# hzykent/LiDAL

Measured on AMD Instinct MI355X. Metric: voxels/sec SPVCNN fwd+bwd @120k pts, higher is better.
Workload: dtype bf16; 1 GPU; spvcnn train step (train.py:127-140: fwd + CE + bwd + Adam), 5 scans x ~120k pts per GPU, 0.05 m voxels, kernel maps rebuilt every step (each step builds the next step's coordinate tables on a second stream; variants.inline_geometry: built inside the forward pass); parallelism=dp1

## Files before the change

### lidal_amd/csrc/voxel.hip

```cpp
#include <cstring>


#include "common.h"

using namespace lidal;

namespace {

typedef __attribute__((ext_vector_type(4))) __bf16 bf16x4_t;

__device__ __forceinline__ float4 ld4(const float* p) { return *reinterpret_cast<const float4*>(p); }
__device__ __forceinline__ float4 ld4(const __bf16* p) {
  bf16x4_t v = *reinterpret_cast<const bf16x4_t*>(p);
  return make_float4((float)v[0], (float)v[1], (float)v[2], (float)v[3]);
}
__device__ __forceinline__ void st4(float* p, float4 v) { *reinterpret_cast<float4*>(p) = v; }
__device__ __forceinline__ void st4(__bf16* p, float4 v) {
  bf16x4_t o;
  o[0] = (__bf16)v.x; o[1] = (__bf16)v.y; o[2] = (__bf16)v.z; o[3] = (__bf16)v.w;
  *reinterpret_cast<bf16x4_t*>(p) = o;
}

template <int VEC>
__device__ __forceinline__ void ldv(const float* p, float (&a)[VEC]) {
// ... 393 lines not shown
  float inv = 1.f;
  if (!DEVOX) { int cv = counts[v]; inv = cv > 0 ? (float)cv : 1.f; }
  float acc[VEC];
#pragma unroll
  for (int u = 0; u < VEC; ++u) acc[u] = 0.f;
  auto add = [&](const float (&x)[VEC], float sc) {
#pragma unroll
    for (int u = 0; u < VEC; ++u) acc[u] += DEVOX ? sc * x[u] : x[u] / inv;
  };
  int64_t j = beg;
  for (; j + 3 < end; j += 4) {
    int e[4]; float sc[4]; float x[4][VEC];
#pragma unroll
    for (int u = 0; u < 4; ++u) e[u] = order[j + u];
#pragma unroll
    for (int u = 0; u < 4; ++u) {
      sc[u] = DEVOX ? w[e[u]] : 1.f;
      ldv<VEC>(src + (int64_t)(DEVOX ? (e[u] >> 3) : e[u]) * c + l * VEC, x[u]);
    }
#pragma unroll
    for (int u = 0; u < 4; ++u) add(x[u], sc[u]);
  }
  for (; j < end; ++j) {
    const int e = order[j];
    float x[VEC];
    ldv<VEC>(src + (int64_t)(DEVOX ? (e >> 3) : e) * c + l * VEC, x);
    add(x, DEVOX ? w[e] : 1.f);
  }
  stv<VEC>(out + v * c + l * VEC, acc);
}

template <typename T>
__global__ void __launch_bounds__(256) segment_fold_kernel(const float* __restrict__ partial,
                                                           T* __restrict__ out, int64_t m, int c,
                                                           int parts) {
  const int cv = c / 4;
  int64_t t = (int64_t)blockIdx.x * 256 + threadIdx.x;
  if (t >= m * cv) return;
  int64_t v = t / cv;
  int j = (int)(t - v * cv) * 4;
  float4 a = ld4(partial + (v * parts) * c + j);
  for (int p = 1; p < parts; ++p) {
    float4 b = ld4(partial + (v * parts + p) * c + j);
    a.x += b.x; a.y += b.y; a.z += b.z; a.w += b.w;
  }
  st4(out + v * c + j, a);
}

static inline int row_lanes(int c, int vec) {
  const int need = (c + vec - 1) / vec;
  int lpr = 4;
  while (lpr < need) lpr <<= 1;
  return lpr > 64 ? 64 : lpr;
}
static inline int segment_vec(int c, int esz) { return (esz == 2 && c % 8 == 0) ? 8 : 4; }
static inline int segment_parts(int64_t n_entries, int64_t m, int c, int esz) {
  if (m <= 0) return 0;
  const int lpr = row_lanes(c, segment_vec(c, esz));
  const int64_t rpw = 64 / lpr, avg = n_entries / m;
  if (avg < 20 * rpw && (m >= 65536 || avg < 8 * rpw)) return 0;
  const int64_t waves = (avg + 16 * rpw - 1) / (16 * rpw);
  int parts = 1;
  while (parts < 4 && (int64_t)parts * 4 < waves) parts <<= 1;
  return parts;
}

constexpr int64_t GROUP_MAX_AVG = 32, GROUP_MAX_AVG_FEW = 12, GROUP_MANY_VOXELS = 65536;

template <typename T, int VEC, bool DEVOX>
void launch_group(const T* src, const int* order, const int64_t* seg_ptr, const float* w, const int* counts,
                  T* out, int64_t m, int c, hipStream_t s) {
  const int need = (c + VEC - 1) / VEC;
#define LIDAL_GROUP(LPR)                                                                               \
  segment_sum_group_kernel<T, LPR, VEC, DEVOX><<<(unsigned)cdiv(m, 256 / LPR), 256, 0, s>>>(src, order, seg_ptr, w, \
                                                                                          counts, out, m, c)
  if (need <= 4) LIDAL_GROUP(4);
  else if (need <= 8) LIDAL_GROUP(8);
  else if (need <= 16) LIDAL_GROUP(16);
  else if (need <= 32) LIDAL_GROUP(32);
  else LIDAL_GROUP(64);
#undef LIDAL_GROUP
}

template <typename T, bool DEVOX>
int launch_segment_sum(const T* src, const int* order, const int64_t* seg_ptr, const float* w,
                       const int* counts, T* out, int64_t m, int c, int64_t n_entries, void* ws,
                       int64_t ws_bytes, hipStream_t s) {
  LIDAL_REQUIRE(c <= 64 * segment_vec(c, (int)sizeof(T)), "segment_sum: at most %d channels per row for this element type",
                64 * segment_vec(c, (int)sizeof(T)));
  if (m > 0 && n_entries / m <= (m >= GROUP_MANY_VOXELS ? GROUP_MAX_AVG : GROUP_MAX_AVG_FEW)) {
    if (sizeof(T) == 2 && c % 8 == 0) launch_group<T, 8, DEVOX>(src, order, seg_ptr, w, counts, out, m, c, s);
    else launch_group<T, 4, DEVOX>(src, order, seg_ptr, w, counts, out, m, c, s);
    LIDAL_CHECK_LAUNCH("segment_sum_group");
    return 0;
  }
  const int parts = segment_parts(n_entries, m, c, (int)sizeof(T));
  float* partial = (float*)ws;
  if (parts > 1)
    LIDAL_REQUIRE(ws != nullptr && ws_bytes >= (int64_t)m * parts * c * 4, "segment_sum workspace too small");
  const bool wide = segment_vec(c, (int)sizeof(T)) == 8;
  const int lpr = row_lanes(c, wide ? 8 : 4);
#define LIDAL_SEG(LPR, VEC)                                                                              \
  do {                                                                                                   \
    if (parts == 0)                                                                                      \
      segment_sum_kernel<T, LPR, VEC, DEVOX><<<(unsigned)cdiv(m, 4), 256, 0, s>>>(src, order, seg_ptr, w, counts, \
                                                                                 out, m, c);             \
    else                                                                                                 \
      segment_sum_wg_kernel<T, LPR, VEC, DEVOX><<<(unsigned)(m * parts), 256, 0, s>>>(                   \
          src, order, seg_ptr, w, counts, out, partial, m, c, parts);                                    \
  } while (0)
  if (wide) {
    if (lpr <= 4) LIDAL_SEG(4, 8); else if (lpr == 8) LIDAL_SEG(8, 8); else if (lpr == 16) LIDAL_SEG(16, 8);
    else if (lpr == 32) LIDAL_SEG(32, 8); else LIDAL_SEG(64, 8);
  } else {
    if (lpr <= 8) LIDAL_SEG(8, 4); else if (lpr == 16) LIDAL_SEG(16, 4); else if (lpr == 32) LIDAL_SEG(32, 4);
    else LIDAL_SEG(64, 4);
  }
#undef LIDAL_SEG
  LIDAL_CHECK_LAUNCH("segment_sum");
  if (parts > 1) {
    segment_fold_kernel<T><<<(unsigned)cdiv(m * (c / 4), 256), 256, 0, s>>>(partial, out, m, c, parts);
    LIDAL_CHECK_LAUNCH("segment_fold");
  }
  return 0;
}

template <typename T, int LPR, int VEC>
__global__ void __launch_bounds__(256) devox_cell_sums_kernel(const T* __restrict__ g, const int* __restrict__ vorder,
                                                              const int64_t* __restrict__ vseg,
                                                              const float* __restrict__ w8, float* __restrict__ cs,
                                                              int64_t m, int c) {
  constexpr int RPW = 64 / LPR;
  __shared__ float red[3][8][LPR * VEC];
  const int lane = threadIdx.x & 63, wave = threadIdx.x >> 6;
  const int l = lane % LPR, grp = lane / LPR;
  const int64_t cell = blockIdx.x;
  const int64_t beg = vseg[cell], end = vseg[cell + 1];
  const int64_t quarter = (end - beg + 3) / 4;
  int64_t b0 = beg + (int64_t)wave * quarter, b1 = b0 + quarter;
  if (b0 > end) b0 = end;
  if (b1 > end) b1 = end;
  float acc[8][VEC];
#pragma unroll
  for (int k = 0; k < 8; ++k)
#pragma unroll
    for (int q = 0; q < VEC; ++q) acc[k][q] = 0.f;
  auto add = [&](const float (&x)[VEC], const float4& wa, const float4& wb) {
    const float wv[8] = {wa.x, wa.y, wa.z, wa.w, wb.x, wb.y, wb.z, wb.w};
#pragma unroll
    for (int k = 0; k < 8; ++k)
      if (wv[k] != 0.f) {
#pragma unroll
        for (int q = 0; q < VEC; ++q) acc[k][q] += wv[k] * x[q];
      }
  };
  for (int64_t base = b0; base < b1; base += 64) {
    const int cnt = (int)((b1 - base < 64) ? (b1 - base) : 64);
    const int mine = lane < cnt ? vorder[base + lane] : 0;
    int ib = 0;
    for (; ib + 4 * RPW <= cnt; ib += 4 * RPW) {
      const int i = ib + grp;
      int p[4]; float x[4][VEC]; float4 wa[4], wb[4];
#pragma unroll
      for (int u = 0; u < 4; ++u) p[u] = __shfl(mine, i + u * RPW, 64);
#pragma unroll
      for (int u = 0; u < 4; ++u) {
        ldv<VEC>(g + (int64_t)p[u] * c + VEC * l, x[u]);
        wa[u] = ld4(w8 + (int64_t)p[u] * 8); wb[u] = ld4(w8 + (int64_t)p[u] * 8 + 4);
      }
#pragma unroll
      for (int u = 0; u < 4; ++u) add(x[u], wa[u], wb[u]);
    }
    for (; ib < cnt; ib += RPW) {
      const int i = ib + grp;
      const bool ok = i < cnt;
      const int p0 = __shfl(mine, ok ? i : 0, 64);
      if (ok) {
        float x0[VEC];
        ldv<VEC>(g + (int64_t)p0 * c + VEC * l, x0);
        add(x0, ld4(w8 + (int64_t)p0 * 8), ld4(w8 + (int64_t)p0 * 8 + 4));
      }
    }
  }
#pragma unroll
  for (int off = LPR; off < 64; off <<= 1) {
#pragma unroll
    for (int k = 0; k < 8; ++k)
#pragma unroll
      for (int q = 0; q < VEC; ++q) acc[k][q] += __shfl_xor(acc[k][q], off, 64);
  }
  if (wave > 0 && grp == 0) {
#pragma unroll
    for (int k = 0; k < 8; ++k)
#pragma unroll
      for (int q = 0; q < VEC; ++q) red[wave - 1][k][l * VEC + q] = acc[k][q];
  }
  __syncthreads();
  if (wave == 0 && grp == 0) {
#pragma unroll
    for (int k = 0; k < 8; ++k) {
      float* dst = cs + ((int64_t)cell * 8 + k) * c + VEC * l;
#pragma unroll
      for (int q = 0; q < VEC; q += 4) {
        float o[4];
#pragma unroll
        for (int e = 0; e < 4; ++e)
          o[e] = ((acc[k][q + e] + red[0][k][l * VEC + q + e]) + red[1][k][l * VEC + q + e]) + red[2][k][l * VEC + q + e];
        st4(dst + q, make_float4(o[0], o[1], o[2], o[3]));
      }
    }
  }
}

template <typename T>
__global__ void __launch_bounds__(256) devox_cell_fold_kernel(const float* __restrict__ cs, const int* __restrict__ corder,
                                                              const int64_t* __restrict__ cseg, T* __restrict__ gin,
                                                              int64_t m, int c) {
  const int cv = c / 4;
  const int64_t t = (int64_t)blockIdx.x * 256 + threadIdx.x;
  if (t >= m * cv) return;
  const int64_t v = t / cv;
  const int jj = (int)(t - v * cv) * 4;
  float4 a = make_float4(0.f, 0.f, 0.f, 0.f);
  for (int64_t i = cseg[v]; i < cseg[v + 1]; ++i) {
    const float4 b = ld4(cs + (int64_t)corder[i] * c + jj);
    a.x += b.x; a.y += b.y; a.z += b.z; a.w += b.w;
  }
  st4(gin + v * c + jj, a);
}

template <typename T>
int launch_devox_cells(const T* g, const int* vorder, const int64_t* vseg, const float* w8, const int* corder,
                       const int64_t* cseg, T* gin, int64_t m, int c, float* cs, hipStream_t s) {
  constexpr int VEC = 16 / (int)sizeof(T);
  const int lpr = c / VEC;
#define LIDAL_CELLS(LPR) devox_cell_sums_kernel<T, LPR, VEC><<<(unsigned)m, 256, 0, s>>>(g, vorder, vseg, w8, cs, m, c)
  if (lpr == 4) LIDAL_CELLS(4); else if (lpr == 8) LIDAL_CELLS(8); else if (lpr == 16) LIDAL_CELLS(16);
  else if (lpr == 32) LIDAL_CELLS(32); else LIDAL_CELLS(64);
#undef LIDAL_CELLS
  LIDAL_CHECK_LAUNCH("devoxelize_bwd_cells(sums)");
  devox_cell_fold_kernel<T><<<(unsigned)cdiv(m * (c / 4), 256), 256, 0, s>>>(cs, corder, cseg, gin, m, c);
  LIDAL_CHECK_LAUNCH("devoxelize_bwd_cells(fold)");
  return 0;
}

}

#define DISPATCH_VEC(kernel, c, total_rows, ...)                                             \
  do {                                                                                       \
    if ((c) % 4 == 0) {                                                                      \
      int64_t t__ = (total_rows) * ((c) / 4);                                                \
      kernel<4><<<(unsigned)cdiv(t__, 256), 256, 0, s>>>(__VA_ARGS__);                       \
    } else {                                                                                 \
      int64_t t__ = (total_rows) * (c);                                                      \
      kernel<1><<<(unsigned)cdiv(t__, 256), 256, 0, s>>>(__VA_ARGS__);                       \
    }                                                                                        \
  } while (0)

#define DISPATCH_TVEC(kernel, T, c, total_rows, ...)                                         \
  do {                                                                                       \
    if (sizeof(T) == 2 && (c) % 8 == 0) {                  \
      int64_t t__ = (total_rows) * ((c) / 8);                                                \
      kernel<T, 8><<<(unsigned)cdiv(t__, 256), 256, 0, s>>>(__VA_ARGS__);                    \
    } else if ((c) % 4 == 0) {                                                                      \
      int64_t t__ = (total_rows) * ((c) / 4);                                                \
      kernel<T, 4><<<(unsigned)cdiv(t__, 256), 256, 0, s>>>(__VA_ARGS__);                    \
    } else {                                                                                 \
      int64_t t__ = (total_rows) * (c);                                                      \
      kernel<T, 1><<<(unsigned)cdiv(t__, 256), 256, 0, s>>>(__VA_ARGS__);                    \
    }                                                                                        \
  } while (0)

extern "C" int lidal_count(const int32_t* idx, int64_t n, int32_t* out, int64_t m, void* stream) {
  hipStream_t s = (hipStream_t)stream;
  if (m > 0) LIDAL_HIP(hipMemsetAsync(out, 0, 4 * m, s));
  if (n == 0 || m == 0) return 0;
  count_kernel<<<(unsigned)cdiv(n, 256), 256, 0, s>>>(idx, n, out, m);
  LIDAL_CHECK_LAUNCH("lidal_count");
  return 0;
}

extern "C" int lidal_voxelize_fwd(const float* feat, const int32_t* idx, const int32_t* counts,
                                  float* out, int64_t n, int64_t m, int c, void* stream) {
  hipStream_t s = (hipStream_t)stream;
  if (m > 0 && c > 0) LIDAL_HIP(hipMemsetAsync(out, 0, 4 * m * c, s));
  if (n == 0 || m == 0 || c == 0) return 0;
  DISPATCH_VEC(voxelize_fwd_kernel, c, n, feat, idx, counts, out, n, m, c);
  LIDAL_CHECK_LAUNCH("lidal_voxelize_fwd");
  return 0;
}

namespace {
template <typename T, int VEC>
__global__ void __launch_bounds__(256) voxelize_1to1_kernel(const T* __restrict__ feat, const int* __restrict__ idx,
                                                            T* __restrict__ out, int64_t n, int c) {
  const int cv = c / VEC;
  const int64_t t = (int64_t)blockIdx.x * blockDim.x + threadIdx.x;
  if (t >= n * cv) return;
  const int64_t i = t / cv;
  const int j = (int)(t - i * cv) * VEC;
  const int pos = idx[i];
  if (pos < 0 || pos >= n) return;
  const T* src = feat + i * c + j;
  T* dst = out + (int64_t)pos * c + j;
#pragma unroll
  for (int v = 0; v < VEC; ++v) dst[v] = src[v];
}
}

extern "C" int lidal_voxelize_fwd_1to1(const void* feat, const int32_t* idx, void* out, int64_t n, int c,
                                       int dtype, void* stream) {
  hipStream_t s = (hipStream_t)stream;
  if (n == 0 || c == 0) return 0;
  if (dtype == LIDAL_F32)
    DISPATCH_TVEC(voxelize_1to1_kernel, float, c, n, (const float*)feat, idx, (float*)out, n, c);
  else if (dtype == LIDAL_BF16)
    DISPATCH_TVEC(voxelize_1to1_kernel, __bf16, c, n, (const __bf16*)feat, idx, (__bf16*)out, n, c);
  else { set_error("voxelize_fwd_1to1: bad dtype %d", dtype); return 2; }
  LIDAL_CHECK_LAUNCH("lidal_voxelize_fwd_1to1");
  return 0;
}

extern "C" int lidal_voxelize_bwd(const void* gout, const int32_t* idx, const int32_t* counts,
                                  const void* residual, void* gin, int64_t n, int64_t m, int c,
                                  int dtype, void* stream) {
  hipStream_t s = (hipStream_t)stream;
  if (n == 0 || c == 0) return 0;
  if (dtype == LIDAL_F32)
    DISPATCH_TVEC(voxelize_bwd_kernel, float, c, n, (const float*)gout, idx, counts,
                  (const float*)residual, (float*)gin, n, m, c);
  else if (dtype == LIDAL_BF16)
    DISPATCH_TVEC(voxelize_bwd_kernel, __bf16, c, n, (const __bf16*)gout, idx, counts,
                  (const __bf16*)residual, (__bf16*)gin, n, m, c);
  else { set_error("voxelize_bwd: bad dtype %d", dtype); return 2; }
  LIDAL_CHECK_LAUNCH("lidal_voxelize_bwd");
  return 0;
}

extern "C" int lidal_devoxelize_fwd(const void* feat, const int32_t* idx, const float* w,
                                    void* out, int64_t n, int64_t m, int c, int dtype,
                                    void* stream) {
  hipStream_t s = (hipStream_t)stream;
  if (n == 0 || c == 0) return 0;
  if (dtype == LIDAL_F32)
    DISPATCH_TVEC(devoxelize_fwd_kernel, float, c, n, (const float*)feat, idx, w, (float*)out, n, m, c);
  else if (dtype == LIDAL_BF16)
    DISPATCH_TVEC(devoxelize_fwd_kernel, __bf16, c, n, (const __bf16*)feat, idx, w, (__bf16*)out, n, m, c);
  else { set_error("devoxelize_fwd: bad dtype %d", dtype); return 2; }
  LIDAL_CHECK_LAUNCH("lidal_devoxelize_fwd");
  return 0;
}

extern "C" int lidal_devoxelize_bwd(const float* gout, const int32_t* idx, const float* w,
                                    float* gin, int64_t n, int64_t m, int c, void* stream) {
  hipStream_t s = (hipStream_t)stream;
  if (m > 0 && c > 0) LIDAL_HIP(hipMemsetAsync(gin, 0, 4 * m * c, s));
  if (n == 0 || m == 0 || c == 0) return 0;
  DISPATCH_VEC(devoxelize_bwd_kernel, c, n, gout, idx, w, gin, n, m, c);
  LIDAL_CHECK_LAUNCH("lidal_devoxelize_bwd");
  return 0;
}

extern "C" int lidal_ti_weights(const float* coords, int cstride, const int64_t* idx, int64_t n,
                                float scale, float* w, int32_t* idx32, void* stream) {
  hipStream_t s = (hipStream_t)stream;
  if (n == 0) return 0;
  LIDAL_REQUIRE(cstride >= 3, "ti_weights: coords need >= 3 columns");
  ti_weights_kernel<<<(unsigned)cdiv(n, 256), 256, 0, s>>>(coords, cstride, idx, n, scale, w, idx32);
  LIDAL_CHECK_LAUNCH("lidal_ti_weights");
  return 0;
}

static int64_t inv_tmp_bytes(int64_t q) { return sort_pairs_ws_bytes(q); }

extern "C" int64_t lidal_invlist_workspace_bytes(int64_t n_entries) {
  int64_t q = n_entries > 0 ? n_entries : 1;
  return 2 * align_up(4 * q, 256) + align_up(4 * q, 256) + align_up(inv_tmp_bytes(q), 256) + 256;
}

extern "C" int lidal_invlist_build(const int32_t* idx, const float* w, int64_t n_entries, int64_t m,
                                   int32_t* order, int64_t* seg_ptr, void* ws, int64_t ws_bytes,
                                   void* stream) {
  hipStream_t s = (hipStream_t)stream;
  LIDAL_REQUIRE(m >= 0 && m < 0x7FFFFFFF, "invlist: bad voxel count");
  if (n_entries == 0) {
    LIDAL_HIP(hipMemsetAsync(seg_ptr, 0, 8 * (m + 1), s));
    return 0;
  }
  LIDAL_REQUIRE(ws_bytes >= lidal_invlist_workspace_bytes(n_entries), "invlist workspace too small");
  int64_t q = n_entries;
  unsigned* keys = (unsigned*)ws;
  unsigned* skeys = (unsigned*)((char*)ws + align_up(4 * q, 256));
  int* vals = (int*)((char*)ws + 2 * align_up(4 * q, 256));
  void* tmp = (char*)ws + 3 * align_up(4 * q, 256);
  inv_keys_kernel<<<(unsigned)cdiv(q, 256), 256, 0, s>>>(idx, w, q, m, keys, vals);
  LIDAL_CHECK_LAUNCH("inv_keys");
  int bits = 1;
  while ((1ll << bits) <= m) ++bits;
  if (int rc = sort_pairs_u32(keys, vals, skeys, order, q, bits, tmp, inv_tmp_bytes(q), s)) return rc;
  inv_segptr_kernel<<<(unsigned)cdiv(m + 1, 256), 256, 0, s>>>(skeys, q, m, seg_ptr);
  LIDAL_CHECK_LAUNCH("inv_segptr");
  return 0;
}

extern "C" int64_t lidal_segment_workspace_bytes(int64_t n_entries, int64_t m, int c) {
  int parts = segment_parts(n_entries, m, c, 2), parts4 = segment_parts(n_entries, m, c, 4);
  if (parts4 > parts) parts = parts4;
  return parts > 1 ? (int64_t)m * parts * c * 4 : 0;
}

extern "C" int lidal_voxelize_fwd_sorted(const void* feat, const int32_t* order,
                                         const int64_t* seg_ptr, const int32_t* counts, void* out,
                                         int64_t m, int c, int dtype, int64_t n_entries, void* ws,
                                         int64_t ws_bytes, void* stream) {
  if (m == 0 || c == 0) return 0;
  LIDAL_REQUIRE(c % 4 == 0, "voxelize_fwd_sorted: channels must be a multiple of 4");
  if (dtype == LIDAL_F32)
    return launch_segment_sum<float, false>((const float*)feat, order, seg_ptr, nullptr, counts,
                                            (float*)out, m, c, n_entries, ws, ws_bytes,
                                            (hipStream_t)stream);
  if (dtype == LIDAL_BF16)
    return launch_segment_sum<__bf16, false>((const __bf16*)feat, order, seg_ptr, nullptr, counts,
                                             (__bf16*)out, m, c, n_entries, ws, ws_bytes,
                                             (hipStream_t)stream);
  set_error("voxelize_fwd_sorted: bad dtype %d", dtype);
  return 2;
}

extern "C" int64_t lidal_devoxelize_bwd_cells_workspace_bytes(int64_t m, int c) { return m * 8 * (int64_t)c * 4; }
extern "C" int lidal_devoxelize_bwd_cells(const void* gout, const int32_t* vorder, const int64_t* vseg, const float* w8,
                                          const int32_t* corder, const int64_t* cseg, void* gin, int64_t m, int c,
                                          int dtype, void* ws, int64_t ws_bytes, void* stream) {
  if (m == 0 || c == 0) return 0;
  const int vec = dtype == LIDAL_F32 ? 4 : 8;
  const int lpr = c / vec;
  LIDAL_REQUIRE(dtype == LIDAL_F32 || dtype == LIDAL_BF16, "devoxelize_bwd_cells: bad dtype %d", dtype);
  LIDAL_REQUIRE(c % vec == 0 && lpr >= 4 && lpr <= 64 && (lpr & (lpr - 1)) == 0,
                "devoxelize_bwd_cells: %d channels (a power of two of 16-byte steps, 4 .. 64 of them)", c);
  LIDAL_REQUIRE(ws != nullptr && ws_bytes >= lidal_devoxelize_bwd_cells_workspace_bytes(m, c), "devoxelize_bwd_cells ws too small");
  if (dtype == LIDAL_F32)
    return launch_devox_cells<float>((const float*)gout, vorder, vseg, w8, corder, cseg, (float*)gin, m, c, (float*)ws,
                                     (hipStream_t)stream);
  return launch_devox_cells<__bf16>((const __bf16*)gout, vorder, vseg, w8, corder, cseg, (__bf16*)gin, m, c, (float*)ws,
                                    (hipStream_t)stream);
}

extern "C" int lidal_devoxelize_bwd_sorted(const void* gout, const int32_t* order,
                                           const int64_t* seg_ptr, const float* w, void* gin,
                                           int64_t m, int c, int dtype, int64_t n_entries, void* ws,
                                           int64_t ws_bytes, void* stream) {
  if (m == 0 || c == 0) return 0;
  LIDAL_REQUIRE(c % 4 == 0, "devoxelize_bwd_sorted: channels must be a multiple of 4");
  if (dtype == LIDAL_F32)
    return launch_segment_sum<float, true>((const float*)gout, order, seg_ptr, w, nullptr,
                                           (float*)gin, m, c, n_entries, ws, ws_bytes,
                                           (hipStream_t)stream);
  if (dtype == LIDAL_BF16)
    return launch_segment_sum<__bf16, true>((const __bf16*)gout, order, seg_ptr, w, nullptr,
                                            (__bf16*)gin, m, c, n_entries, ws, ws_bytes,
                                            (hipStream_t)stream);
  set_error("devoxelize_bwd_sorted: bad dtype %d", dtype);
  return 2;
}
```

### lidal_amd/network/plan.py

```python
import array
import ctypes
import os
import struct

import torch

from .. import backend as B
from ..nn.functional import conv as _C
from ..nn.functional import norm as _N
from ..nn.functional import devoxelize as _DV
from ..nn.functional.invlist import inverse_lists
from ..nn.functional.voxelize import _index32

__all__ = ['planned_forward', 'enabled', 'COUNTERS']

ENABLED = os.environ.get('LIDAL_PLAN', '1') != '0'
BN_SUMS = None

OP_CONV_WEIGHT_IMAGE_BATCH, OP_CONV_APPLY_IMAGE, OP_CONV_DGRAD_BN_SUMS, OP_CONV_WGRAD = 1, 2, 3, 4
OP_BN_TRAIN_FWD, OP_BN_TRAIN_FWD_TILES, OP_BN_BWD, OP_BN_BWD_TILES, OP_BN_EVAL_FWD, OP_BN_FOLD = 5, 6, 7, 8, 9, 10
OP_COLSUM, OP_ADD_RELU_FWD, OP_ADD_RELU_BWD, OP_VOXELIZE_FWD_1TO1, OP_VOXELIZE_FWD_SORTED = 11, 12, 13, 14, 15
OP_VOXELIZE_BWD, OP_DEVOXELIZE_FWD, OP_DEVOXELIZE_BWD_SORTED, OP_CE_FWD, OP_CE_BWD = 16, 17, 18, 19, 20
OP_COPY2D, OP_ADD2D, OP_TRANSPOSE_F32, OP_CAST_ROWS_BF16, OP_VIEW_MEAN_SOFTMAX = 21, 22, 23, 24, 25
OP_FORK_SIDE, OP_JOIN_SIDE, OP_CONV_APPLY_IMAGE_WS, OP_CONV_DGRAD_BN_SUMS_WS = 26, 27, 28, 29
# ... 878 lines not shown
        self.w += (OP_CONV_WGRAD | flag, x, g, n, n, 0, self.koff[n], 0, gw, sc, slabs, 1, ca, cb, wcode)
        self.nops += 1
        if not direct:
            self.w += (OP_TRANSPOSE_F32 | flag, gw, cb, self.slot(c.w), ca, c.co)
            self.nops += 1
        if not need_gx:
            return 0
        gx = self.galloc(n * ca * self.esz)
        self.w += (OP_CONV_APPLY_IMAGE | branch, g, c.img_b, 0, 0, 0, gx, n, n, cb, ca, 1, 0, self.code, 0, 0, 0, 0, 0)
        self.nops += 1
        return gx

    def b_colsum(self, g, n, c, out, flag=0):
        nb = _bn_ws(n, c) + 12 * c
        self.w += (OP_COLSUM | flag, g, self.code, n, c, out, self.scratch(nb, flag), nb)
        self.nops += 1

    def b_conv_bn(self, cb, g, g_stride, n_in, n_out, tables, need_gx=True, ci=None):
        c, r = cb
        x, x1, mean, invstd = self.saved[id(cb)]
        dx = self.b_bn(r, x1, n_out, mean, invstd, g, g_stride)
        if c.transposed:
            rules, table, n_gin, kflip = tables[6:8], tables[0:3], n_in, 0
        elif c.strided:
            rules, table, n_gin, kflip = tables[6:8], tables[3:6], n_in, 0
        else:
            rules, table, n_gin, kflip = tables[3:8], tables[0:3], n_in, 1
        self.b_wgrad(c, x, n_in, dx, n_out, rules, ci)
        if not need_gx:
            return 0
        return self.b_dgrad(c, dx, n_out, table, n_gin, kflip)[0]

    def b_res(self, r, g, n, k3):
        x, x1, mean1, inv1, y1, x2, mean2, inv2, out, xs, means, invs = self.saved[id(r)]
        co = r.c2.co
        gm = self.galloc(n * co * self.esz)
        part2 = parts = nb = 0
        sums2 = sumss = nparts = 0
        if _N.tail_tiles(n, self.dtype):
            nparts = int(B.lib().lidal_bn_tail_parts(n, co, self.code))
            sums2 = self.galloc(co * nparts * 8)
            sumss = self.galloc(co * nparts * 8) if r.cs is not None else 0
            self.w += (OP_ADD_RELU_BWD_BN_TILE_SUMS, out, g, gm, self.code, n, co, x2, mean2, inv2, sums2,
                       xs if sumss else 0, means if sumss else 0, invs if sumss else 0, sumss, nparts)
        elif _N.tail_sums(n):
            nb = _bn_ws(n, co)
            part2 = self.galloc(nb)
            parts = self.galloc(nb) if r.cs is not None else 0
            self.w += (OP_ADD_RELU_BWD_BN_SUMS, out, g, gm, self.code, n, co, x2, mean2, inv2, part2,
                       xs if parts else 0, means if parts else 0, invs if parts else 0, parts, nb)
        else:
            self.w += (OP_ADD_RELU_BWD, out, g, gm, n * co, self.code)
        self.nops += 1
        fl = 0
        if r.cs is not None:
            fl = self.fork(2) if (BRANCH_ROWS and n >= BRANCH_ROWS and (self.bf16 or not F32_BN_ALONE)) else 0
            dxs = self.b_bn(r.bs, xs, n, means, invs, gm, co, sumss, None, flag=fl, part=(parts, nb), nparts=nparts)
            g_skip = self.b_dense(r.cs, x, n, dxs, co, branch=fl)
        else:
            g_skip = gm
        dx2 = self.b_bn(r.b2, x2, n, mean2, inv2, gm, co, sums2, 0, part=(part2, nb), nparts=nparts)
        table, rules = k3[0:3], k3[3:8]
        self.b_wgrad(r.c2, y1, n, dx2, n, rules)
        p = self.ptr
        bnb = (x1, mean1, inv1, p[r.b1.w], p[r.b1.b], 1) if self.bn_sums else None
        dy1, sums = self.b_dgrad(r.c2, dx2, n, table, n, 1, 0, bnb)
        dx1 = self.b_bn(r.b1, x1, n, mean1, inv1, dy1, r.c1.co, sums)
        self.b_wgrad(r.c1, x, n, dx1, n, rules)
        if fl:
            self.join(2)
        return self.b_dgrad(r.c1, dx1, n, table, n, 1, g_skip)[0]

    def b_add(self, a, a_stride, b, b_stride, n, c):
        out = self.galloc(n * c * self.esz)
        self.w += (OP_ADD2D, a, a_stride, b, b_stride, out, c, n, c, self.code)
        self.nops += 1
        return out

    def b_devox(self, g, lvl, c):
        t = self.T.pt[lvl]
        P, m = self.T.p, self.T.n[lvl]
        gin = self.galloc(m * c * self.esz)
        if t[9] is not None:
            nb = m * 8 * c * 4
            self.w += (OP_DEVOXELIZE_BWD_CELLS, g, t[9][0], t[9][1], t[6], t[9][2], t[9][3], gin, m, c, self.code,
                       self.scratch(nb), nb)
            self.nops += 1
            return gin
        nb = _seg_ws(8 * P, m, c)
        self.w += (OP_DEVOXELIZE_BWD_SORTED, g, t[7], t[8], t[6], gin, m, c, self.code, 8 * P,
                   self.scratch(nb) if nb else 0, nb)
        self.nops += 1
        return gin

    def b_vox(self, g, lvl, c, skip):
        t = self.T.pt[lvl]
        P, m = self.T.p, self.T.n[lvl]
        gin = self.galloc(P * c * self.esz)
        self.w += (OP_VOXELIZE_BWD, g, t[0], t[1], skip, gin, P, m, c, self.code)
        self.nops += 1
        return gin

    def b_point(self, pt, g, need_gx=True, flag=0):
        lin, r = pt
        P = self.T.p
        z_in, x1, mean, invstd = self.saved[id(pt)]
        dx = self.b_bn(r, x1, P, mean, invstd, g, lin.co, flag=flag)
        gx = self.b_dense(lin.conv, z_in, P, dx, lin.co, need_gx, True, branch=flag)
        self.b_colsum(dx, P, lin.co, self.slot(lin.b), flag)
        return gx

    def point_fork(self):
        return self.fork(POINT_SIDE) if (POINT_SIDE and self.bf16) else 0

    def point_join(self):
        if POINT_SIDE and POINT_SIDE in self.open:
            self.join(POINT_SIDE)

    def b_dropout(self, which, g, n, c):
        noise = self.noise[which]
        if noise is None:
            return g
        self.flush()
        gt = self.barena.tensor(g, (n, c), self.dtype)
        if isinstance(noise, int):
            gt.zero_()
        else:
            torch.mul(gt, noise, out=gt)
        return g

    def backward(self, g_logits, g_feat):
        if self.done:
            raise RuntimeError('lidal_amd.plan: this step has already run its backward pass (its activations are '
                               'released; retain_graph is not supported by the planned step)')
        if not self.geometry.alive():
            raise RuntimeError('lidal_amd: this backward pass reads the coordinate tables of a geometry that is stale -- two '
                               'newer ones have been submitted to its prefetcher since (queue forward AND backward of a '
                               'batch before the second submit() after its own: network/geometry.py GeometryPrefetcher)')
        prog, T = self.prog, self.T
        n, k3, k2 = T.n, T.k3, T.k2
        e = self.esz
        self.stream = B.stream()
        self.barena = _Arena(self.dev)
        flat = torch.empty(prog.flat_numel + 16, dtype=torch.float32, device=self.dev)
        self.flat = flat.data_ptr()
        assert self.flat % 16 == 0
        lin = prog.classifier
        x, rows, co_pad = self.saved['cls']
        g = g_logits
        if g.dtype != self.dtype or not g.is_contiguous():
            g = g.contiguous().to(self.dtype)
        gp = self.galloc(rows * co_pad * e)
        self.w += (OP_COPY2D, g.data_ptr(), lin.co * e, gp, co_pad * e, rows, lin.co * e, (co_pad - lin.co) * e)
        self.nops += 1
        gy = self.b_dense(lin.conv, x, rows, gp, co_pad, True, True)
        self.b_colsum(gp, rows, co_pad, self.slot(lin.b))
        c_out = self.c_feat
        if g_feat is not None:
            gf = g_feat if (g_feat.dtype == self.dtype and g_feat.is_contiguous()) else g_feat.contiguous().to(self.dtype)
            self.keep_gf = gf
            gy = self.b_add(gy, c_out, gf.data_ptr(), c_out, rows, c_out)
        gz_lin = 0
        if prog.spvcnn:
            gz_lin = self.b_point(prog.points[2], gy, flag=self.point_fork())
            gy = self.b_devox(gy, 0, c_out)
        g_skip = [0] * 5
        for i in (3, 2, 1, 0):
# ... 183 lines not shown
```

Before: 29.41 million voxels/s.

## Balance segment-sum and devox-cell reductions with fixed-size entry chunks per wave

Replaces the per-segment work split (one block per cell, or m*parts blocks) with a chunked scheme. Each wave handles a fixed 64-entry span of the sorted list, locates its starting segment by a wave-wide binary search, and walks across segment boundaries. Partial sums for segments that span chunks go to a workspace and are combined by a separate fold kernel. It is applied to both the mean voxelize path with long segments and the devoxelize-backward cell sums, so load stays balanced when segment sizes are skewed. The cost is more complex boundary handling, an extra fold pass over spilled partials, and a doubled cell workspace.

```diff
diff --git a/lidal_amd/csrc/voxel.hip b/lidal_amd/csrc/voxel.hip
--- a/lidal_amd/csrc/voxel.hip
+++ b/lidal_amd/csrc/voxel.hip
@@ -499,19 +499,30 @@
 #undef LIDAL_GROUP
 }
 
+static inline bool segment_chunked(int64_t n_entries, int64_t m) {
+  return m > 0 && n_entries / m > (m >= GROUP_MANY_VOXELS ? GROUP_MAX_AVG : GROUP_MAX_AVG_FEW);
+}
+
+template <typename T>
+int launch_chunk_mean(const T* src, const int* order, const int64_t* seg_ptr, const int* counts, T* out, int64_t m, int c,
+                      int64_t n_entries, void* ws, int64_t ws_bytes, hipStream_t s);
+
 template <typename T, bool DEVOX>
 int launch_segment_sum(const T* src, const int* order, const int64_t* seg_ptr, const float* w,
                        const int* counts, T* out, int64_t m, int c, int64_t n_entries, void* ws,
                        int64_t ws_bytes, hipStream_t s) {
   LIDAL_REQUIRE(c <= 64 * segment_vec(c, (int)sizeof(T)), "segment_sum: at most %d channels per row for this element type",
                 64 * segment_vec(c, (int)sizeof(T)));
-  if (m > 0 && n_entries / m <= (m >= GROUP_MANY_VOXELS ? GROUP_MAX_AVG : GROUP_MAX_AVG_FEW)) {
+  if (m > 0 && !segment_chunked(n_entries, m)) {
     if (sizeof(T) == 2 && c % 8 == 0) launch_group<T, 8, DEVOX>(src, order, seg_ptr, w, counts, out, m, c, s);
     else launch_group<T, 4, DEVOX>(src, order, seg_ptr, w, counts, out, m, c, s);
     LIDAL_CHECK_LAUNCH("segment_sum_group");
     return 0;
   }
   const int parts = segment_parts(n_entries, m, c, (int)sizeof(T));
+  if constexpr (!DEVOX) {
+    if (parts >= 1) return launch_chunk_mean<T>(src, order, seg_ptr, counts, out, m, c, n_entries, ws, ws_bytes, s);
+  }
   float* partial = (float*)ws;
   if (parts > 1)
     LIDAL_REQUIRE(ws != nullptr && ws_bytes >= (int64_t)m * parts * c * 4, "segment_sum workspace too small");
@@ -522,8 +533,8 @@
     if (parts == 0)                                                                                      \
       segment_sum_kernel<T, LPR, VEC, DEVOX><<<(unsigned)cdiv(m, 4), 256, 0, s>>>(src, order, seg_ptr, w, counts, \
                                                                                  out, m, c);             \
-    else                                                                                                 \
-      segment_sum_wg_kernel<T, LPR, VEC, DEVOX><<<(unsigned)(m * parts), 256, 0, s>>>(                   \
+    else if constexpr (DEVOX)                                                                            \
+      segment_sum_wg_kernel<T, LPR, VEC, true><<<(unsigned)(m * parts), 256, 0, s>>>(                    \
           src, order, seg_ptr, w, counts, out, partial, m, c, parts);                                    \
   } while (0)
   if (wide) {
@@ -542,105 +553,286 @@
   return 0;
 }
 
-template <typename T, int LPR, int VEC>
-__global__ void __launch_bounds__(256) devox_cell_sums_kernel(const T* __restrict__ g, const int* __restrict__ vorder,
-                                                              const int64_t* __restrict__ vseg,
-                                                              const float* __restrict__ w8, float* __restrict__ cs,
-                                                              int64_t m, int c) {
-  constexpr int RPW = 64 / LPR;
-  __shared__ float red[3][8][LPR * VEC];
-  const int lane = threadIdx.x & 63, wave = threadIdx.x >> 6;
+constexpr int CHUNK_SHIFT = 6, CHUNK = 1 << CHUNK_SHIFT;
+
+__device__ __forceinline__ int cells_chunk_shift(int64_t n, int64_t m) {
+  int s = CHUNK_SHIFT;
+  while (((n + ((int64_t)1 << s) - 1) >> s) > m) ++s;
+  return s;
+}
+
+__device__ __forceinline__ int wave_lower_bound(const int64_t* __restrict__ seg, int len, int64_t key, int lane) {
+  int lo = 0;
+  while (len > 0) {
+    const int step = (len + 63) >> 6;
+    const int64_t i = (int64_t)lo + (int64_t)(lane + 1) * step - 1;
+    const bool less = i < (int64_t)lo + len && seg[i] < key;
+    const int nless = __popcll(__ballot(less));
+    const int end = lo + len;
+    lo += nless * step;
+    len = end - lo < step - 1 ? end - lo : step - 1;
+  }
+  return lo;
+}
+
+template <typename T, int VEC>
+struct row_piece {
+  static constexpr bool PACKED = sizeof(T) * VEC == 16;
+  uint4 raw;
+  float f[PACKED ? 1 : VEC];
+  __device__ __forceinline__ void load(const T* p) {
+    if constexpr (PACKED) raw = *reinterpret_cast<const uint4*>(p);
+    else { float t[VEC]; ldv<VEC>(p, t);
+#pragma unroll
+      for (int q = 0; q < VEC; ++q) f[q] = t[q]; }
+  }
+  __device__ __forceinline__ void unpack(float (&a)[VEC]) const {
+    if constexpr (PACKED && sizeof(T) == 4) {
+      a[0] = __uint_as_float(raw.x); a[1] = __uint_as_float(raw.y); a[2] = __uint_as_float(raw.z); a[3] = __uint_as_float(raw.w);
+    } else if constexpr (PACKED) {
+      const unsigned q4[4] = {raw.x, raw.y, raw.z, raw.w};
+#pragma unroll
+      for (int v = 0; v < 4; ++v) {
+        a[2 * v] = __uint_as_float(q4[v] << 16);
+        a[2 * v + 1] = __uint_as_float(q4[v] & 0xFFFF0000u);
+      }
+    } else {
+#pragma unroll
+      for (int q = 0; q < VEC; ++q) a[q] = f[q];
+    }
+  }
+};
+
+template <typename T, int LPR, int VEC, bool CELLS>
+__global__ void __launch_bounds__(256) chunk_sums_kernel(const T* __restrict__ src, const int* __restrict__ order,
+                                                         const int64_t* __restrict__ seg, const float* __restrict__ w8,
+                                                         const int* __restrict__ counts, T* __restrict__ out,
+                                                         float* __restrict__ part, int* __restrict__ meta, int64_t m64, int c) {
+  constexpr int RPW = 64 / LPR, ROWS = CELLS ? 8 : 1;
+  const int lane = threadIdx.x & 63;
   const int l = lane % LPR, grp = lane / LPR;
-  const int64_t cell = blockIdx.x;
-  const int64_t beg = vseg[cell], end = vseg[cell + 1];
-  const int64_t quarter = (end - beg + 3) / 4;
-  int64_t b0 = beg + (int64_t)wave * quarter, b1 = b0 + quarter;
-  if (b0 > end) b0 = end;
-  if (b1 > end) b1 = end;
-  float acc[8][VEC];
-#pragma unroll
-  for (int k = 0; k < 8; ++k)
-#pragma unroll
-    for (int q = 0; q < VEC; ++q) acc[k][q] = 0.f;
-  auto add = [&](const float (&x)[VEC], const float4& wa, const float4& wb) {
-    const float wv[8] = {wa.x, wa.y, wa.z, wa.w, wb.x, wb.y, wb.z, wb.w};
-#pragma unroll
-    for (int k = 0; k < 8; ++k)
-      if (wv[k] != 0.f) {
-#pragma unroll
-        for (int q = 0; q < VEC; ++q) acc[k][q] += wv[k] * x[q];
+  const bool act = VEC * l < c;
+  const int m = (int)m64;
+  const int64_t n64 = seg[m];
+  const int n = (int)n64;
+  const int shift = CELLS ? cells_chunk_shift(n64, m64) : CHUNK_SHIFT;
+  int nch = (int)((n64 + ((int64_t)1 << shift) - 1) >> shift);
+  if (nch < 1) nch = 1;
+  const int k = __builtin_amdgcn_readfirstlane((int)(blockIdx.x * 4 + (threadIdx.x >> 6)));
+  if (k >= nch) return;
+  const bool last = k == nch - 1;
+  const int cb = k << shift;
+  const int ce = last ? n : cb + (1 << shift);
+  const int own_hi = last ? 0x7FFFFFFF : ce;
+
+  int wbase = 0, win = 0, cwin = 1;
+  auto fill = [&](int v) {
+    wbase = v;
+    const int i = v + lane < m ? v + lane : m;
+    win = (int)seg[i];
+    if (!CELLS) cwin = counts[i < m ? i : m - 1];
+  };
+  int cur, cur_beg = 0, cur_end = 0x7FFFFFFF;
+  float inv = 1.f;
+  auto look = [&]() {
+    if (cur >= m) { cur_end = 0x7FFFFFFF; return; }
+    if (cur + 1 - wbase > 63) fill(cur);
+    cur_beg = __builtin_amdgcn_readlane(win, cur - wbase);
+    cur_end = __builtin_amdgcn_readlane(win, cur + 1 - wbase);
+    if (!CELLS) { const int cv = __builtin_amdgcn_readlane(cwin, cur - wbase); inv = cv > 0 ? (float)cv : 1.f; }
+  };
+  {
+    const int v_lo = __builtin_amdgcn_readfirstlane(wave_lower_bound(seg, m + 1, cb, lane));
+    fill(v_lo > 0 ? v_lo - 1 : 0);
+    cur = (v_lo > 0 && __builtin_amdgcn_readlane(win, v_lo - wbase) > cb) ? v_lo - 1 : v_lo;
+    look();
+  }
+
+  float acc[ROWS][VEC];
+#pragma unroll
+  for (int r = 0; r < ROWS; ++r)
+#pragma unroll
+    for (int q = 0; q < VEC; ++q) acc[r][q] = 0.f;
+
+  auto flush = [&](bool whole) {
+#pragma unroll
+    for (int r = 0; r < ROWS; ++r) {
+#pragma unroll
+      for (int off = LPR; off < 64; off <<= 1)
+#pragma unroll
+        for (int q = 0; q < VEC; ++q) acc[r][q] += __shfl_xor(acc[r][q], off, 64);
+      __builtin_amdgcn_sched_barrier(0);
+    }
+    const bool own = cur_beg >= cb;
+    if constexpr (CELLS) {
+      float* dst = part + (int64_t)(own ? cur : m + k) * 8 * c + VEC * l;
+#pragma unroll
+      for (int r = 0; r < 8; ++r)
+        if (grp == (r & (RPW - 1)) && act) {
+#pragma unroll
+          for (int q = 0; q < VEC; q += 4) st4(dst + (int64_t)r * c + q, make_float4(acc[r][q], acc[r][q + 1], acc[r][q + 2], acc[r][q + 3]));
+        }
+    } else {
+      if (grp == 0 && act) {
+        if (own && whole) stv<VEC>(out + (int64_t)cur * c + VEC * l, acc[0]);
+        else {
+          float* dst = part + ((int64_t)k * 2 + (own ? 0 : 1)) * c + VEC * l;
+#pragma unroll
+          for (int q = 0; q < VEC; q += 4) st4(dst + q, make_float4(acc[0][q], acc[0][q + 1], acc[0][q + 2], acc[0][q + 3]));
+        }
       }
+    }
+#pragma unroll
+    for (int r = 0; r < ROWS; ++r)
+#pragma unroll
+      for (int q = 0; q < VEC; ++q) acc[r][q] = 0.f;
   };
-  for (int64_t base = b0; base < b1; base += 64) {
-    const int cnt = (int)((b1 - base < 64) ? (b1 - base) : 64);
-    const int mine = lane < cnt ? vorder[base + lane] : 0;
-    int ib = 0;
-    for (; ib + 4 * RPW <= cnt; ib += 4 * RPW) {
-      const int i = ib + grp;
-      int p[4]; float x[4][VEC]; float4 wa[4], wb[4];
-#pragma unroll
-      for (int u = 0; u < 4; ++u) p[u] = __shfl(mine, i + u * RPW, 64);
+  auto next_cell = [&]() { cur_beg = cur_end; ++cur; look(); };
+
+  for (int base = cb; base < ce; base += 64) {
+    const int cnt = ce - base < 64 ? ce - base : 64;
+    const int mine = lane < cnt ? order[base + lane] : -1;
+    float wr[ROWS];
+    if constexpr (CELLS) {
+      float4 wa = make_float4(0.f, 0.f, 0.f, 0.f), wb = wa;
+      if (mine >= 0) { wa = ld4(w8 + (int64_t)mine * 8); wb = ld4(w8 + (int64_t)mine * 8 + 4); }
+      wr[0] = wa.x; wr[1] = wa.y; wr[2] = wa.z; wr[3] = wa.w; wr[4] = wb.x; wr[5] = wb.y; wr[6] = wb.z; wr[7] = wb.w;
+    } else {
+      wr[0] = mine >= 0 ? 1.f : 0.f;
+    }
+    for (int ib = 0; ib < cnt; ib += 4 * RPW) {
+      row_piece<T, VEC> raw[4];
 #pragma unroll
       for (int u = 0; u < 4; ++u) {
-        ldv<VEC>(g + (int64_t)p[u] * c + VEC * l, x[u]);
-        wa[u] = ld4(w8 + (int64_t)p[u] * 8); wb[u] = ld4(w8 + (int64_t)p[u] * 8 + 4);
+        const int e = __shfl(mine, ib + u * RPW + grp, 64);
+        raw[u].load((e >= 0 && act) ? src + (int64_t)e * c + VEC * l : reinterpret_cast<const T*>(g_zero_row));
       }
 #pragma unroll
-      for (int u = 0; u < 4; ++u) add(x[u], wa[u], wb[u]);
-    }
-    for (; ib < cnt; ib += RPW) {
-      const int i = ib + grp;
-      const bool ok = i < cnt;
-      const int p0 = __shfl(mine, ok ? i : 0, 64);
-      if (ok) {
-        float x0[VEC];
-        ldv<VEC>(g + (int64_t)p0 * c + VEC * l, x0);
-        add(x0, ld4(w8 + (int64_t)p0 * 8), ld4(w8 + (int64_t)p0 * 8 + 4));
+      for (int u = 0; u < 4; ++u) {
+        const int r0 = base + ib + u * RPW;
+        if (r0 < ce) {
+          const int r1 = r0 + RPW < ce ? r0 + RPW : ce;
+          const int pos = r0 + grp;
+          float x[VEC], sc[ROWS];
+          raw[u].unpack(x);
+#pragma unroll
+          for (int r = 0; r < ROWS; ++r) sc[r] = __shfl(wr[r], ib + u * RPW + grp, 64);
+          bool plain = true;
+#pragma unroll
+          for (int r = 0; r < ROWS; ++r) plain = plain && sc[r] != 0.f;
+          auto add = [&](bool on) {
+            if (__all(on && plain)) {
+#pragma unroll
+              for (int r = 0; r < ROWS; ++r)
+#pragma unroll
+                for (int q = 0; q < VEC; ++q) acc[r][q] += CELLS ? sc[r] * x[q] : x[q] / inv;
+            } else {
+#pragma unroll
+              for (int r = 0; r < ROWS; ++r) {
+                if (on && sc[r] != 0.f) {
+#pragma unroll
+                  for (int q = 0; q < VEC; ++q) acc[r][q] += CELLS ? sc[r] * x[q] : x[q] / inv;
+                }
+                __builtin_amdgcn_sched_barrier(0);
+              }
+            }
+          };
+          while (cur_end < r1) {
+            add(pos >= cur_beg && pos < cur_end);
+            flush(true);
+            next_cell();
+          }
+          add(pos >= cur_beg);
+        }
       }
     }
   }
-#pragma unroll
-  for (int off = LPR; off < 64; off <<= 1) {
-#pragma unroll
-    for (int k = 0; k < 8; ++k)
-#pragma unroll
-      for (int q = 0; q < VEC; ++q) acc[k][q] += __shfl_xor(acc[k][q], off, 64);
-  }
-  if (wave > 0 && grp == 0) {
-#pragma unroll
-    for (int k = 0; k < 8; ++k)
-#pragma unroll
-      for (int q = 0; q < VEC; ++q) red[wave - 1][k][l * VEC + q] = acc[k][q];
-  }
-  __syncthreads();
-  if (wave == 0 && grp == 0) {
-#pragma unroll
-    for (int k = 0; k < 8; ++k) {
-      float* dst = cs + ((int64_t)cell * 8 + k) * c + VEC * l;
-#pragma unroll
-      for (int q = 0; q < VEC; q += 4) {
-        float o[4];
-#pragma unroll
-        for (int e = 0; e < 4; ++e)
-          o[e] = ((acc[k][q + e] + red[0][k][l * VEC + q + e]) + red[1][k][l * VEC + q + e]) + red[2][k][l * VEC + q + e];
-        st4(dst + q, make_float4(o[0], o[1], o[2], o[3]));
-      }
-    }
-  }
+  while (cur < m && cur_end <= ce && cur_beg < own_hi) { flush(true); next_cell(); }
+  const bool tail = cur < m && cur_beg < own_hi;
+  if (!CELLS && lane == 0) {
+    meta[2 * k] = tail && cur_beg >= cb ? cur : -1;
+    meta[2 * k + 1] = cur_end;
+  }
+  if (tail) flush(false);
+}
+
+template <typename T>
+__global__ void __launch_bounds__(256) span_fold_kernel(const float* __restrict__ part, const int* __restrict__ meta,
+                                                        const int64_t* __restrict__ seg, T* __restrict__ out, int64_t m,
+                                                        int64_t chunks, int c) {
+  const int cv = c / 4;
+  const int64_t t = (int64_t)blockIdx.x * 256 + threadIdx.x;
+  const int64_t nch = (seg[m] + CHUNK - 1) >> CHUNK_SHIFT;
+  if (t >= chunks * cv) return;
+  const int64_t k = t / cv;
+  if (k >= nch) return;
+  const int j = (int)(t - k * cv) * 4;
+  const int v = meta[2 * k];
+  if (v < 0) return;
+  const int64_t k1 = ((int64_t)meta[2 * k + 1] - 1) >> CHUNK_SHIFT;
+  float4 a = ld4(part + (k * 2) * c + j);
+  for (int64_t kk = k + 1; kk <= k1; ++kk) {
+    const float4 b = ld4(part + (kk * 2 + 1) * c + j);
+    a.x += b.x; a.y += b.y; a.z += b.z; a.w += b.w;
+  }
+  st4(out + (int64_t)v * c + j, a);
+}
+
+static inline int64_t chunk_ws_bytes(int64_t n_entries, int c) {
+  const int64_t chunks = n_entries > 0 ? (n_entries + CHUNK - 1) / CHUNK : 1;
+  return align_up(chunks * 2 * c * 4, 256) + chunks * 8;
+}
+
+template <typename T>
+int launch_chunk_mean(const T* src, const int* order, const int64_t* seg_ptr, const int* counts, T* out, int64_t m, int c,
+                      int64_t n_entries, void* ws, int64_t ws_bytes, hipStream_t s) {
+  LIDAL_REQUIRE(m < 0x7FFFFFFF && n_entries < 0x7FFFFFFF, "segment_sum: list too long");
+  LIDAL_REQUIRE(ws != nullptr && ws_bytes >= chunk_ws_bytes(n_entries, c), "segment_sum workspace too small");
+  const int64_t chunks = n_entries > 0 ? (n_entries + CHUNK - 1) / CHUNK : 1;
+  float* part = (float*)ws;
+  int* meta = (int*)((char*)ws + align_up(chunks * 2 * c * 4, 256));
+  const bool wide = segment_vec(c, (int)sizeof(T)) == 8;
+  const int lpr = row_lanes(c, wide ? 8 : 4);
+#define LIDAL_CHUNK(LPR, VEC)                                                                                          \
+  chunk_sums_kernel<T, LPR, VEC, false><<<(unsigned)cdiv(chunks, 4), 256, 0, s>>>(src, order, seg_ptr, nullptr, counts, out, \
+                                                                                  part, meta, m, c)
+  if (wide) {
+    if (lpr <= 4) LIDAL_CHUNK(4, 8); else if (lpr == 8) LIDAL_CHUNK(8, 8); else if (lpr == 16) LIDAL_CHUNK(16, 8);
+    else if (lpr == 32) LIDAL_CHUNK(32, 8); else LIDAL_CHUNK(64, 8);
+  } else {
+    if (lpr <= 4) LIDAL_CHUNK(4, 4); else if (lpr <= 8) LIDAL_CHUNK(8, 4); else if (lpr == 16) LIDAL_CHUNK(16, 4);
+    else if (lpr == 32) LIDAL_CHUNK(32, 4); else LIDAL_CHUNK(64, 4);
+  }
+#undef LIDAL_CHUNK
+  LIDAL_CHECK_LAUNCH("segment_sum(chunks)");
+  span_fold_kernel<T><<<(unsigned)cdiv(chunks * (c / 4), 256), 256, 0, s>>>(part, meta, seg_ptr, out, m, chunks, c);
+  LIDAL_CHECK_LAUNCH("segment_sum(span fold)");
+  return 0;
 }
 
 template <typename T>
 __global__ void __launch_bounds__(256) devox_cell_fold_kernel(const float* __restrict__ cs, const int* __restrict__ corder,
-                                                              const int64_t* __restrict__ cseg, T* __restrict__ gin,
+                                                              const int64_t* __restrict__ cseg,
+                                                              const int64_t* __restrict__ vseg, T* __restrict__ gin,
                                                               int64_t m, int c) {
   const int cv = c / 4;
   const int64_t t = (int64_t)blockIdx.x * 256 + threadIdx.x;
   if (t >= m * cv) return;
   const int64_t v = t / cv;
   const int jj = (int)(t - v * cv) * 4;
+  const int shift = cells_chunk_shift(vseg[m], m);
   float4 a = make_float4(0.f, 0.f, 0.f, 0.f);
   for (int64_t i = cseg[v]; i < cseg[v + 1]; ++i) {
-    const float4 b = ld4(cs + (int64_t)corder[i] * c + jj);
+    const int e = corder[i];
+    const int64_t cell = e >> 3;
+    float4 b = ld4(cs + (int64_t)e * c + jj);
+    const int64_t beg = vseg[cell], end = vseg[cell + 1];
+    if (end > beg) {
+      for (int64_t k = (beg >> shift) + 1; k <= ((end - 1) >> shift); ++k) {
+        const float4 h = ld4(cs + ((m + k) * 8 + (e & 7)) * c + jj);
+        b.x += h.x; b.y += h.y; b.z += h.z; b.w += h.w;
+      }
+    }
     a.x += b.x; a.y += b.y; a.z += b.z; a.w += b.w;
   }
   st4(gin + v * c + jj, a);
@@ -651,12 +843,14 @@
                        const int64_t* cseg, T* gin, int64_t m, int c, float* cs, hipStream_t s) {
   constexpr int VEC = 16 / (int)sizeof(T);
   const int lpr = c / VEC;
-#define LIDAL_CELLS(LPR) devox_cell_sums_kernel<T, LPR, VEC><<<(unsigned)m, 256, 0, s>>>(g, vorder, vseg, w8, cs, m, c)
+#define LIDAL_CELLS(LPR)                                                                                             \
+  chunk_sums_kernel<T, LPR, VEC, true><<<(unsigned)cdiv(m, 4), 256, 0, s>>>(g, vorder, vseg, w8, nullptr, nullptr, cs, \
+                                                                            nullptr, m, c)
   if (lpr == 4) LIDAL_CELLS(4); else if (lpr == 8) LIDAL_CELLS(8); else if (lpr == 16) LIDAL_CELLS(16);
   else if (lpr == 32) LIDAL_CELLS(32); else LIDAL_CELLS(64);
 #undef LIDAL_CELLS
   LIDAL_CHECK_LAUNCH("devoxelize_bwd_cells(sums)");
-  devox_cell_fold_kernel<T><<<(unsigned)cdiv(m * (c / 4), 256), 256, 0, s>>>(cs, corder, cseg, gin, m, c);
+  devox_cell_fold_kernel<T><<<(unsigned)cdiv(m * (c / 4), 256), 256, 0, s>>>(cs, corder, cseg, vseg, gin, m, c);
   LIDAL_CHECK_LAUNCH("devoxelize_bwd_cells(fold)");
   return 0;
 }
@@ -823,7 +1017,9 @@
 extern "C" int64_t lidal_segment_workspace_bytes(int64_t n_entries, int64_t m, int c) {
   int parts = segment_parts(n_entries, m, c, 2), parts4 = segment_parts(n_entries, m, c, 4);
   if (parts4 > parts) parts = parts4;
-  return parts > 1 ? (int64_t)m * parts * c * 4 : 0;
+  const int64_t split = parts > 1 ? (int64_t)m * parts * c * 4 : 0;
+  const int64_t chunked = segment_chunked(n_entries, m) && parts >= 1 ? chunk_ws_bytes(n_entries, c) : 0;
+  return split > chunked ? split : chunked;
 }
 
 extern "C" int lidal_voxelize_fwd_sorted(const void* feat, const int32_t* order,
@@ -844,7 +1040,7 @@
   return 2;
 }
 
-extern "C" int64_t lidal_devoxelize_bwd_cells_workspace_bytes(int64_t m, int c) { return m * 8 * (int64_t)c * 4; }
+extern "C" int64_t lidal_devoxelize_bwd_cells_workspace_bytes(int64_t m, int c) { return 2 * m * 8 * (int64_t)c * 4; }
 extern "C" int lidal_devoxelize_bwd_cells(const void* gout, const int32_t* vorder, const int64_t* vseg, const float* w8,
                                           const int32_t* corder, const int64_t* cseg, void* gin, int64_t m, int c,
                                           int dtype, void* ws, int64_t ws_bytes, void* stream) {
@@ -855,6 +1051,7 @@
   LIDAL_REQUIRE(c % vec == 0 && lpr >= 4 && lpr <= 64 && (lpr & (lpr - 1)) == 0,
                 "devoxelize_bwd_cells: %d channels (a power of two of 16-byte steps, 4 .. 64 of them)", c);
   LIDAL_REQUIRE(ws != nullptr && ws_bytes >= lidal_devoxelize_bwd_cells_workspace_bytes(m, c), "devoxelize_bwd_cells ws too small");
+  LIDAL_REQUIRE(m < 0x3FFFFFFF, "devoxelize_bwd_cells: too many cells");
   if (dtype == LIDAL_F32)
     return launch_devox_cells<float>((const float*)gout, vorder, vseg, w8, corder, cseg, (float*)gin, m, c, (float*)ws,
                                      (hipStream_t)stream);
diff --git a/lidal_amd/network/plan.py b/lidal_amd/network/plan.py
--- a/lidal_amd/network/plan.py
+++ b/lidal_amd/network/plan.py
@@ -984,7 +984,7 @@
         P, m = self.T.p, self.T.n[lvl]
         gin = self.galloc(m * c * self.esz)
         if t[9] is not None:
-            nb = m * 8 * c * 4
+            nb = int(B.lib_handle().lidal_devoxelize_bwd_cells_workspace_bytes(m, c))
             self.w += (OP_DEVOXELIZE_BWD_CELLS, g, t[9][0], t[9][1], t[6], t[9][2], t[9][3], gin, m, c, self.code,
                        self.scratch(nb), nb)
             self.nops += 1
```

After: 29.57 million voxels/s (median of 6 runs). Within noise of the previous version (+0.6%).
